# remit0/SpeechRecognitionProject

Measured on AMD Instinct MI355X. Metric: utterances/sec (1 s @16 kHz) MFCC+CNN-BiGRU train step, higher is better.
Workload: dtype fp32; 1 GPU; cfg2 mfcc_bgru: on-device MFCC[39x51] + 2-layer BiGRU(512) + FC, CE, backward, Adam (full training.py step), per-GPU batch 256; model=mfcc_bgru, global_batch=256, clip_samples=16000, parallelism=dp1, step_execution=HIP graph replay of the whole step, sync_bn=False

## Files before the change

include/srk.h:

```cpp
#ifndef SRK_H_
#define SRK_H_

#include <stdint.h>

#define SRK_ABI_VERSION 3

#ifdef __cplusplus
extern "C" {
#endif

enum srk_status {
  SRK_OK = 0,
  SRK_ERR_INVALID = -1,
  SRK_ERR_HIP = -2,
  SRK_ERR_INTERNAL = -3,
  SRK_ERR_TIMEOUT = -4,
};

int srk_version(void);
const char* srk_source_stamp(void);
const char* srk_last_error(void);
int srk_init(int device);
int64_t srk_scratch_generation(void);
int srk_prof_enable(int on);
// ... 54 lines not shown
                        float* rowsum, void* stream);
int srk_gemm_16(int trans_a, int trans_b, int64_t M, int64_t N, int64_t K, float alpha, const uint16_t* A,
                int64_t lda, const uint16_t* B, int64_t ldb, float beta, float* C, int64_t ldc,
                const float* bias, int bias_mode, void* stream);
int srk_gemm_16_batched(int trans_a, int trans_b, int64_t M, int64_t N, int64_t K, float alpha,
                        const uint16_t* A, int64_t lda, int64_t sA, const uint16_t* B, int64_t ldb,
                        int64_t sB, float beta, float* C, int64_t ldc, int64_t sC, int batch, void* stream);
int srk_colsum_f32(const float* X, int64_t M, int64_t N, int64_t ldx, float* out, float beta, void* stream);
int srk_gemm_plan_describe(int trans_a, int trans_b, int64_t M, int64_t N, int64_t K, int64_t lda, int64_t ldb,
                           int64_t ldc, int batch, int64_t sA, int64_t sB, int64_t sC, int bias_mode, int has_rowsum,
                           int operands16, int prec, int no_split, int plan_batch, uint64_t a_addr, uint64_t b_addr,
                           uint64_t c_addr, uint64_t bias_addr, char* buf, int64_t cap);
int srk_gemm_pack_plan(int64_t K, int64_t slab, int64_t first, int64_t stride, int64_t count, int64_t* blocks,
                       int64_t blocks_cap, int64_t* slab_counts, int64_t slabs_cap, int64_t* n_slabs,
                       int64_t* packed_slab);

int64_t srk_gru_workspace_floats(int64_t B, int64_t T, int64_t in, int64_t H, int backward);
int srk_gru_layer_fwd(const float* x, int64_t B, int64_t T, int64_t in, int64_t H, const float* w_ih,
                      const float* w_hh, const float* b_ih, const float* b_hh, float* y, float* ws,
                      void* stream);
int srk_gru_layer_bwd(const float* x, int64_t B, int64_t T, int64_t in, int64_t H, const float* w_ih,
                      const float* w_hh, const float* y, const float* ws_fwd, const float* dy, float* dx,
                      float* dw_ih, float* dw_hh, float* db_ih, float* db_hh, int accumulate, float* ws,
                      void* stream);
int64_t srk_gru_y16_offset(int64_t B, int64_t T, int64_t in, int64_t H);
int srk_gru_layer_fwd_x16(const float* x, const void* x16, int64_t B, int64_t T, int64_t in, int64_t H,
                          const float* w_ih, const float* w_hh, const float* b_ih, const float* b_hh, float* y,
                          float* ws, void* stream);
int srk_gru_layer_bwd_x16(const float* x, const void* x16, int64_t B, int64_t T, int64_t in, int64_t H,
                          const float* w_ih, const float* w_hh, const float* y, const float* ws_fwd, const float* dy,
// ... 157 lines not shown
```

speechrecognitionproject_amd/_lib.py:

```python
import contextlib
import ctypes
import os
import re

import torch

_HERE = os.path.dirname(os.path.abspath(__file__))
LIB_PATH = os.environ.get("SRK_LIB") or os.path.join(_HERE, "libsrk.so")
HEADER = os.path.join(os.path.dirname(_HERE), "include", "srk.h")
ABI_VERSION = 3

_P = ctypes.c_void_p
_I64 = ctypes.c_int64
_I = ctypes.c_int
_F = ctypes.c_float
_D = ctypes.c_double

_SIGS = {
    "srk_version": [],
    "srk_last_error": [],
    "srk_init": [_I],
    "srk_prof_enable": [_I],
    "srk_prof_read": [ctypes.c_char_p, ctypes.POINTER(ctypes.c_int64), ctypes.POINTER(ctypes.c_double),
                      ctypes.POINTER(ctypes.c_double)],
# ... 25 lines not shown
    "srk_augment": [_P, _I64, _P, _I64, _P, _P, _P, _P, ctypes.c_uint64, _P, _P],
    "srk_pitch_workspace_bytes": [_I64],
    "srk_pitch_shift": [_P, _I64, _P, _P, _I64, _P, _P, _I64, _P],
    "srk_wav_read_batch": [ctypes.POINTER(ctypes.c_char_p), _I64, _P, _P, _I],
    "srk_softmax_ensemble": [_P, _I64, _I64, _I64, _P, _P, _P, _P],
    "srk_gemm_f32": [_I, _I, _I64, _I64, _I64, _F, _P, _I64, _P, _I64, _F, _P, _I64, _P, _I, _P],
    "srk_gemm_rowsum_f32": [_I, _I, _I64, _I64, _I64, _F, _P, _I64, _P, _I64, _F, _P, _I64, _P, _P],
    "srk_gemm_16": [_I, _I, _I64, _I64, _I64, _F, _P, _I64, _P, _I64, _F, _P, _I64, _P, _I, _P],
    "srk_gemm_16_batched": [_I, _I, _I64, _I64, _I64, _F, _P, _I64, _I64, _P, _I64, _I64, _F, _P, _I64, _I64, _I, _P],
    "srk_colsum_f32": [_P, _I64, _I64, _I64, _P, _F, _P],
    "srk_gemm_plan_describe": [_I, _I, _I64, _I64, _I64, _I64, _I64, _I64, _I, _I64, _I64, _I64, _I, _I, _I, _I, _I, _I,
                               ctypes.c_uint64, ctypes.c_uint64, ctypes.c_uint64, ctypes.c_uint64, ctypes.c_char_p,
                               _I64],
    "srk_gemm_pack_plan": [_I64, _I64, _I64, _I64, _I64, ctypes.POINTER(_I64), _I64, ctypes.POINTER(_I64), _I64,
                           ctypes.POINTER(_I64), ctypes.POINTER(_I64)],
    "srk_gru_workspace_floats": [_I64, _I64, _I64, _I64, _I],
    "srk_gru_layer_fwd": [_P, _I64, _I64, _I64, _I64, _P, _P, _P, _P, _P, _P, _P],
    "srk_gru_layer_bwd": [_P, _I64, _I64, _I64, _I64, _P, _P, _P, _P, _P, _P, _P, _P, _P, _P, _I, _P, _P],
    "srk_gru_y16_offset": [_I64, _I64, _I64, _I64],
    "srk_gru_layer_fwd_x16": [_P, _P, _I64, _I64, _I64, _I64, _P, _P, _P, _P, _P, _P, _P],
    "srk_gru_layer_bwd_x16": [_P, _P, _I64, _I64, _I64, _I64, _P, _P, _P, _P, _P, _P, _P, _P, _P, _P, _I, _P, _P],
    "srk_gru_top_last_workspace_floats": [_I64, _I64, _I64, _I64, _I],
    "srk_gru_top_last_fwd": [_P, _P, _I64, _I64, _I64, _I64, _P, _P, _P, _P, _P, _P, _P, _P, _P],
    "srk_gru_top_last_bwd": [_P, _P, _I64, _I64, _I64, _I64, _P, _P, _P, _P, _P, _I, _P, _P, _P, _P, _P, _I, _P, _P],
    "srk_conv2d_workspace_floats": [_I64, _I64, _I64, _I64],
    "srk_conv2d_nhwc_fwd": [_P, _I64, _I64, _I64, _I64, _P, _P, _I64, _I64, _I64, _I64, _I64, _I64, _I64, _P, _P,
                            _P],
    "srk_conv2d_nhwc_bwd": [_P, _I64, _I64, _I64, _I64, _P, _I64, _I64, _I64, _I64, _I64, _I64, _I64, _P, _P, _P,
                            _P, _P, _P],
    "srk_conv2d_nhwc_fwd16": [_P, _I64, _I64, _I64, _I64, _P, _P, _I64, _I64, _I64, _I64, _I64, _I64, _I64, _P, _P,
# ... 129 lines not shown
def gemm_pack_plan(K, slab, first, stride, count):
    n = max(int(count), 0)
    ns = max(-(-int(K) // int(slab)), 0) if slab > 0 else 0
    blocks = (_I64 * max(n, 1))()
    counts = (_I64 * max(ns, 1))()
    n_slabs, pslab = _I64(0), _I64(0)
    call("srk_gemm_pack_plan", K, slab, first, stride, count, blocks, n, counts, ns, ctypes.byref(n_slabs),
         ctypes.byref(pslab))
    out, at = [], 0
    for s in range(n_slabs.value):
        out.append([int(b) for b in blocks[at:at + counts[s]]])
        at += counts[s]
    return out, int(pslab.value)


def scratch_generation():
    return int(lib().srk_scratch_generation())


PRECISIONS = {"fp32": 0, "bf16": 1, "fp16": 2}
_precision = "fp32"


def set_option(name, value):
    global _precision
    call("srk_set_option", name.encode(), int(value))
    if name == "matmul_precision":
        _precision = next(k for k, v in PRECISIONS.items() if v == int(value))


# ... 87 lines not shown
```

speechrecognitionproject_amd/csrc/gemm.h:

```cpp
#pragma once
#include "srk_internal.h"

namespace srk {

struct GemmDesc {
  int64_t M = 0, N = 0, K = 0;
  const float* A = nullptr; int64_t lda = 0; bool ta = false;
  const float* B = nullptr; int64_t ldb = 0; bool tb = false;
  float* C = nullptr; int64_t ldc = 0;
  float alpha = 1.f, beta = 0.f;
  const float* bias = nullptr; int bias_mode = 0;
  int batch = 1; int64_t sA = 0, sB = 0, sC = 0;
  float* rowsum = nullptr; float rowsum_beta = 0.f;
  int64_t sRS = 0;
  int prec = -1;
  const uint16_t* A16 = nullptr;
  const uint16_t* B16 = nullptr;
  bool no_split = false;
  int plan_batch = 0;
  int64_t plan_M = 0;
  int pin_splits = 0;
  int64_t pin_kchunk = 0;
};

int gemm_f32(const GemmDesc& d, hipStream_t stream);

bool gemm_f32_pin_as(const GemmDesc& full, GemmDesc& part);

bool gemm_f32_p32_split(const GemmDesc& d, int* splits, int64_t* kchunk);

constexpr int kGemmGroupMax = 4;
int gemm_f32_group(const GemmDesc* ds, int n, hipStream_t stream);
bool gemm_group_enabled();

struct PackPlan {
  int64_t K = 0, slab = 0, first = 0, stride = 0, count = 0;
  int64_t nslabs = 0, pslab = 0;
  __host__ __device__ int64_t lo(int64_t s) const {
    const int64_t k0 = s * slab;
    if (s >= nslabs) return count;
    if (k0 <= first) return 0;
    const int64_t b = (k0 - first + stride - 1) / stride;
    return b < count ? b : count;
  }
  __host__ __device__ int64_t src(int64_t kp, bool* live) const {
    const int64_t s = kp / pslab, r = kp - s * pslab, b = lo(s) + (r >> 3);
    *live = false;
    if (b >= lo(s + 1)) return -1;
// ... 15 lines not shown
```

speechrecognitionproject_amd/csrc/gemm.hip:

```cpp
#include <algorithm>
#include <cstdlib>
#include <type_traits>

#include "gemm.h"
#include "mfma_tile.h"

namespace srk {
namespace {

using namespace tile;

struct KernelArgs {
  GemmDesc d;
  int tiles_m, tiles_n;
  int tiles;
  int nblk;
  int group_m;
  int remap;
  int64_t kchunk;
  float* partial;
  float* rs_partial;
  int sk_wgs;
  int sk_ki;
  float* sk_slab;
};

__device__ __forceinline__ void tile_of(int t, int tiles_m, int tiles_n, int group_m, int& tm, int& tn) {
  const int gsz_full = group_m * tiles_n;
  const int grp = t / gsz_full, first_m = grp * group_m;
  const int gm = tiles_m - first_m < group_m ? tiles_m - first_m : group_m;
  const int tin = t - grp * gsz_full;
  tm = first_m + tin % gm;
  tn = tin / gm;
}
__device__ __forceinline__ int64_t sk_begin(int64_t w, int64_t total, int64_t W) { return w * total / W; }
__device__ __forceinline__ int sk_owner(int64_t it, int64_t total, int64_t W) { return (int)(((it + 1) * W - 1) / total); }

template <int TM, int TN>
__device__ __forceinline__ void store_acc(const KernelArgs& ka, const f32x16 (&acc)[TM][TN], int split, int64_t m0,
                                          int64_t n0, int wm0, int wn0, int lane, int64_t z) {
  const GemmDesc& d = ka.d;
  const int lh = lane >> 5, lc = lane & 31;
  const bool split_mode = ka.partial != nullptr;
#pragma unroll
  for (int i = 0; i < TM; ++i) {
#pragma unroll
    for (int j = 0; j < TN; ++j) {
      const int64_t col = n0 + wn0 + j * 32 + lc;
      if (col >= d.N) continue;
#pragma unroll
      for (int r = 0; r < 16; ++r) {
// ... 1081 lines not shown
  return ((double)d.M * (double)d.K * esz + (double)d.K * (double)d.N * esz + c) * (double)d.batch;
}

constexpr int kP32BK = 16;
template <bool KC>
struct P32Half {
  static constexpr int FLOATS = 128 * kP32BK;
  __device__ static __forceinline__ v4f frag(const float* img, int r0, int kb, int lane) {
    const int row = r0 + (lane & 31), h = lane >> 5;
    if (KC) return *reinterpret_cast<const v4f*>(img + row * kP32BK + (((2 * kb + h) ^ ((row >> 2) & 3)) << 2));
    const float* q = img + (8 * kb + 4 * h) * 128 + row;
    return v4f{q[0], q[128], q[256], q[384]};
  }
  __device__ static __forceinline__ void src(int piece, int lane, int64_t r0, int64_t rows, int64_t ld, unsigned& voff,
                                             int& kk, bool& row_ok) {
    const int p = piece * 64 + lane;
    if (KC) {
      const int row = p >> 2, kc = (p & 3) ^ ((row >> 2) & 3);
      voff = (unsigned)(((r0 + row) * ld + kc * 4) * 4);
      kk = kc * 4;
      row_ok = r0 + row < rows;
    } else {
      const int k = p >> 5, u = p & 31;
      voff = (unsigned)((k * ld + r0 + u * 4) * 4);
      kk = k;
      row_ok = r0 + u * 4 < rows;
    }
  }
  __device__ static __forceinline__ int64_t kstep_bytes(int64_t ld) { return KC ? 4 : 4 * ld; }
};

template <bool TA, bool TB>
__device__ __forceinline__ void gemm_p32_body(const KernelArgs& ka, const int blk, const int64_t z) {
  constexpr int BK = kP32BK, NST = 4;
  constexpr bool AKC = !TA, BKC = TB;
  using HA = P32Half<AKC>;
  using HB = P32Half<BKC>;
  constexpr int HALF = HA::FLOATS;
  constexpr int STAGE = 4 * HALF;
  __shared__ __attribute__((aligned(1024))) float smem[NST * STAGE];
  typedef __attribute__((address_space(3))) void* lds_ptr;
  auto bar = [] {
    asm volatile("" ::: "memory");
    __builtin_amdgcn_s_barrier();
    asm volatile("" ::: "memory");
// ... 7 lines not shown
    int lin = blk;
    if (ka.remap) {
      const int b = blk, xcd = b & 7, q = ka.nblk >> 3, r = ka.nblk & 7;
      lin = (xcd < r ? xcd * (q + 1) : r * (q + 1) + (xcd - r) * q) + (b >> 3);
    }
    sk_it = sk_begin(lin, sk_total, ka.sk_wgs);
    sk_end = sk_begin(lin + 1, sk_total, ka.sk_wgs);
  }
  for (bool first_seg = true;; first_seg = false) {
  int split = 0, tm, tn;
  int64_t kb0, ke;
  float* seg_slab = nullptr;
  if (sk) {
    if (sk_it >= sk_end) break;
    const int t = (int)(sk_it / ka.sk_ki);
    const int64_t t0 = (int64_t)t * ka.sk_ki, kt_end = min((int64_t)ka.sk_ki, sk_end - t0);
    kb0 = (sk_it - t0) * BK;
    ke = min(d.K, kt_end * BK);
    tile_of(t, ka.tiles_m, ka.tiles_n, ka.group_m, tm, tn);
    const int w0 = sk_owner(t0, sk_total, ka.sk_wgs), w1 = sk_owner(t0 + ka.sk_ki - 1, sk_total, ka.sk_wgs);
    const int wme = sk_owner(sk_it, sk_total, ka.sk_wgs);
    if (w1 > w0) seg_slab = ka.sk_slab + (int64_t)(wme - w0) * d.M * d.N;
    sk_it = t0 + ka.sk_ki;
    if (!first_seg) __syncthreads();
  } else {
    if (!first_seg) break;
    map_tile_at(blk, ka.nblk, ka.tiles, ka.tiles_m, ka.tiles_n, ka.group_m, ka.remap != 0, split, tm, tn);
    kb0 = split * ka.kchunk;
    ke = (kb0 + ka.kchunk < d.K) ? kb0 + ka.kchunk : d.K;
  }
  const int64_t m0 = (int64_t)tm * 256, n0 = (int64_t)tn * 256;
  const int nk = ke > kb0 ? (int)((ke - kb0 + BK - 1) / BK) : 0;

  typedef unsigned u32x4s __attribute__((ext_vector_type(4)));
  auto rsrc32 = [](const float* p) {
    const uint64_t a = (uint64_t)(uintptr_t)p;
    return u32x4s{(unsigned)__builtin_amdgcn_readfirstlane((unsigned)a),
                  (unsigned)__builtin_amdgcn_readfirstlane((unsigned)(a >> 32)), 0x7ffffff0u, 0x00020000u};
// ... 64 lines not shown
#pragma unroll
    for (int q = 0; q < BK / 8; ++q) {
      v4f fa[4], fb[2];
#pragma unroll
      for (int i = 0; i < 4; ++i) fa[i] = HA::frag(As, i * 32, q, lane);
#pragma unroll
      for (int j = 0; j < 2; ++j) fb[j] = HB::frag(Bs, bc0 + j * 32, q, lane);
      if (tn_ < nk) {
        if (q == 0) dma_a(tn_);
        else dma_b(tn_);
      }
      if (q == BK / 8 - 1) retire_keep(min(nk - 1 - (kt + 1), NST - 2));
      asm volatile("s_waitcnt lgkmcnt(0)" ::: "memory");
      bar();
      __builtin_amdgcn_s_setprio(1);
#pragma unroll
      for (int ss = 0; ss < 4; ++ss)
#pragma unroll
        for (int i = 0; i < 4; ++i)
#pragma unroll
          for (int j = 0; j < 2; ++j) acc[i][j] = __builtin_amdgcn_mfma_f32_32x32x2f32(fa[i][ss], fb[j][ss], acc[i][j], 0, 0, 0);
      __builtin_amdgcn_s_setprio(0);
      if (do_rs) {
#pragma unroll
        for (int i = 0; i < 4; ++i) rs[i] += (fa[i][0] + fa[i][1]) + (fa[i][2] + fa[i][3]);
      }
      bar();
    }
  }
  if (grp == 0) bar();

  pp_epilogue(ka, acc, smem, split, m0, n0, grp, wc, wave, lane, z, seg_slab);
  if (do_rs) {
    const int splits = ka.nblk / ka.tiles;
    float* rsum = d.rowsum + z * d.sRS;
#pragma unroll
// ... 24 lines not shown
  const int b = (int)blockIdx.x;
  int i = 0;
#pragma unroll
  for (int j = 1; j < kGemmGroupMax; ++j)
    if (j < ga.n && b >= ga.first[j]) i = j;
  const int blk = b - ga.first[i];
  if (blk >= ga.m[i].nblk) return;
  gemm_p32_body<TA, TB>(ga.m[i], blk, 0);
}

constexpr int kSkFixupSlices = 8;
__global__ __launch_bounds__(256) void sk_fixup_kernel(KernelArgs ka) {
  const GemmDesc& d = ka.d;
  const int t = blockIdx.x / kSkFixupSlices, slice = blockIdx.x - t * kSkFixupSlices;
  const int64_t total = (int64_t)ka.tiles * ka.sk_ki, t0 = (int64_t)t * ka.sk_ki;
  const int w0 = sk_owner(t0, total, ka.sk_wgs), w1 = sk_owner(t0 + ka.sk_ki - 1, total, ka.sk_wgs);
  if (w1 == w0) return;
  int tm, tn;
  tile_of(t, ka.tiles_m, ka.tiles_n, ka.group_m, tm, tn);
  const int nseg = w1 - w0 + 1;
  const int64_t MN = d.M * d.N;
  const bool vec = d.N % 4 == 0 && d.ldc % 4 == 0 && (uintptr_t)d.C % 16 == 0 && (uintptr_t)ka.sk_slab % 16 == 0 &&
                   (d.bias_mode != 1 || (uintptr_t)d.bias % 16 == 0);
  constexpr int ROWS = 256 / kSkFixupSlices, ITEMS = ROWS * 64 / 256;
  const int64_t r0 = (int64_t)tm * 256 + slice * ROWS;
  if (vec) {
    v4f v[ITEMS];
    int64_t off[ITEMS];
    bool ok[ITEMS];
#pragma unroll
    for (int u = 0; u < ITEMS; ++u) {
// ... 30 lines not shown
    const int64_t row = r0 + (i >> 6), col = (int64_t)tn * 256 + (i & 63) * 4;
    if (row >= d.M || col >= d.N) continue;
    const int64_t o = row * d.N + col;
#pragma unroll
    for (int e = 0; e < 4; ++e) {
      if (col + e >= d.N) break;
      float v = 0.f;
      for (int g = 0; g < nseg; ++g) v += ka.sk_slab[g * MN + o + e];
      v *= d.alpha;
      if (d.bias_mode == 1) v += d.bias[col + e];
      else if (d.bias_mode == 2) v += d.bias[row];
      float* c = d.C + row * d.ldc + col + e;
      if (d.beta != 0.f) v += d.beta * *c;
      *c = v;
    }
  }
}

__global__ __launch_bounds__(256) void splitk_reduce_kernel(GemmDesc d, const float* __restrict__ partial, int splits) {
  const int64_t i = (int64_t)blockIdx.x * blockDim.x + threadIdx.x;
  if (i >= d.M * d.N) return;
  partial += (int64_t)blockIdx.y * splits * d.M * d.N;
  d.C += (int64_t)blockIdx.y * d.sC;
  const int64_t row = i / d.N, col = i % d.N;
  float s = 0.f;
#pragma unroll 8
  for (int k = 0; k < splits; ++k) s += partial[(int64_t)k * d.M * d.N + i];
  float v = d.alpha * s;
  if (d.bias_mode == 1) v += d.bias[col];
  else if (d.bias_mode == 2) v += d.bias[row];
// ... 477 lines not shown
  part.pin_kchunk = pf.ka.kchunk;
  if (gemm_plan(part, pp) == SRK_OK && pp.family == pf.family && pp.bk == pf.bk && pp.prec == pf.prec) return true;
  part.pin_splits = 0;
  part.pin_kchunk = 0;
  return false;
}

bool gemm_f32_p32_split(const GemmDesc& d, int* splits, int64_t* kchunk) {
  GemmPlan p;
  if (gemm_plan(d, p) != SRK_OK || p.family != kFamP32 || p.streamk) return false;
  *splits = p.splits;
  *kchunk = p.ka.kchunk;
  return true;
}

int gemm_f32_group(const GemmDesc* ds, int n, hipStream_t s) {
  SRK_REQUIRE(ds && n >= 1 && n <= kGemmGroupMax, SRK_ERR_INVALID, "gemm_group: 1 .. %d members", kGemmGroupMax);
  GemmPlan plans[kGemmGroupMax];
  int order[kGemmGroupMax];
  for (int i = 0; i < n; ++i) {
    if (int rc = gemm_plan(ds[i], plans[i])) return rc;
    SRK_REQUIRE(plans[i].family == kFamP32 && !plans[i].streamk && ds[i].batch == 1 && ds[i].ta == ds[0].ta &&
                    ds[i].tb == ds[0].tb,
                SRK_ERR_INVALID, "gemm_group: member %d is not a batch-1, non-stream-K gemm_p32_kernel launch of the "
                "group's (ta, tb)", i);
    order[i] = i;
  }
  const auto klen = [&](int i) { return std::min(plans[i].ka.kchunk, std::max<int64_t>(ds[i].K, 1)); };
  std::stable_sort(order, order + n, [&](int a, int b) { return klen(a) > klen(b); });
  size_t off[kGemmGroupMax], need = 0;
// ... 162 lines not shown
    for (int64_t r = 0; r < p.pslab; r += 8) {
      bool live;
      const int64_t row = p.src(s * p.pslab + r, &live);
      if (row < 0) continue;
      SRK_REQUIRE(nb < blocks_cap, SRK_ERR_INTERNAL, "gemm_pack_plan: more kept blocks than live rows");
      blocks[nb++] = row / 8;
      ++slab_counts[s];
    }
  }
  *n_slabs = p.nslabs;
  *packed_slab = p.pslab;
  return SRK_OK;
  SRK_API_END
}

extern "C" int srk_gemm_plan_describe(int trans_a, int trans_b, int64_t M, int64_t N, int64_t K, int64_t lda,
                                      int64_t ldb, int64_t ldc, int batch, int64_t sA, int64_t sB, int64_t sC,
                                      int bias_mode, int has_rowsum, int operands16, int prec, int no_split,
                                      int plan_batch, uint64_t a_addr, uint64_t b_addr, uint64_t c_addr,
                                      uint64_t bias_addr, char* buf, int64_t cap) {
  SRK_API_BEGIN
  SRK_REQUIRE(buf && cap > 0, SRK_ERR_INVALID, "gemm_plan_describe: no buffer");
  buf[0] = 0;
  srk::GemmDesc d;
  d.M = M; d.N = N; d.K = K;
  d.lda = lda; d.ta = trans_a != 0;
  d.ldb = ldb; d.tb = trans_b != 0;
  if (operands16) {
    d.A16 = reinterpret_cast<const uint16_t*>(a_addr); d.B16 = reinterpret_cast<const uint16_t*>(b_addr);
  } else {
// ... 18 lines not shown
```

speechrecognitionproject_amd/csrc/gru.hip:

```cpp
#include <algorithm>

#include "gemm.h"
#include "gru_internal.h"

namespace srk {
namespace {

constexpr int kRows = 64;
constexpr int kUnits = 16;
constexpr int kBK = 128;
constexpr int kPitch = kBK + 4;

struct GruArgs {
  int B, T, H, in;
  int G, S;
  const float* y_in;
  float* y;
  const float* gi;
  const float* w_hh;
  const float* b_hh;
  float* gates;
  const float* dy;
  float* dgi;
  float* dgh;
// ... 698 lines not shown
  const int64_t ld = h16 ? in8_of(in) : srk::pad4(in);
  const bool pad = ld != in;
  float* wpad = pad && !h16 ? ws + L.wpad : nullptr;
  float* dwpad = pad ? ws + (h16 ? L.dwpad8 : L.dwpad) : nullptr;
  float* dxpad = pad ? ws + (h16 ? L.dxpad8 : L.dxpad) : nullptr;
  Mat m_dgi{dgi, nullptr}, m_dgh{dgh, nullptr}, m_x{pad ? ws_fwd + F.xpad : x, nullptr},
      m_w{pad ? wpad : w_ih, nullptr}, m_y{y, nullptr};
  if (h16) {
    m_dgi = {nullptr, u16(ws + L.dgi)};
    m_dgh = {nullptr, u16(ws + L.dgh16)};
    m_x = {nullptr, x16_in ? static_cast<const uint16_t*>(x16_in) : u16(ws_fwd + F.x16)};
    m_w = {nullptr, u16(ws_fwd + F.w16)};
    m_y = {nullptr, u16(ws_fwd + F.y16)};
  }
  int rc;
  const int dw_parts = h16 ? path.bwd.dw_parts : 0;
  if (path.persistent) {
    srk::GruPArgs p = rec_args(B, T, H, w_hh, ws, L);
    p.y_in = y; p.gates = gates; p.dy = dy;
    if (h16) {
      p.dgi16 = const_cast<uint16_t*>(m_dgi.h); p.dgh16 = const_cast<uint16_t*>(m_dgh.h); p.dbias = ws + L.part;
      if (dw_parts) {
        if ((rc = srk::g_gs.get((size_t)dw_parts * 2 * 3 * H * H, &p.dw_part))) return rc;
        p.y16_in = m_y.h;
      }
    } else {
      p.dgi = dgi; p.dgh = dgh; p.dgh_edge = dgh_edge;
      p.one_dir = top_last >= 2 ? 1 : 0;
    }
    if ((rc = srk::gru_persistent_launch(p, path.bwd, true, s))) return rc;
    if (h16) {
      const int prows = path.bwd.bias_part_rows, bparts = (int)((B + 255) / 256 * (256 / prows));
      if (dw_parts) {
        const int64_t per_dir = 3 * H * H, n4 = 2 * per_dir / 4;
        const int dw_blocks = (int)((n4 + 255) / 256);
        srk::ProfScope prof("gru_dwhh_reduce", s, 4.0 * (dw_parts + 2) * 2 * per_dir);
        hipLaunchKernelGGL(srk::dwhh_dbias_reduce_kernel, dim3((unsigned)(dw_blocks + (6 * H + 255) / 256)), dim3(256),
                           0, s, p.dw_part, dw_parts, (int)B, per_dir, dw_hh, (int)accumulate, dw_blocks, p.dbias,
                           bparts, (int)H, prows, db_ih, db_hh);
        SRK_CHECK_HIP(hipGetLastError());
      } else if ((rc = srk::launch256(srk::dbias_reduce_kernel, 6 * H, s, p.dbias, bparts, B, H, prows, db_ih, db_hh,
                                      accumulate))) {
        return rc;
      }
    }
    if (top_last == 3 && (rc = srk::launch256(srk::zero_cols_kernel, BT * 3 * H / 4, s, dgi, BT, 3 * H, 3 * H, 6 * H)))
      return rc;
    if (top_last >= 2 && (rc = srk::launch256(srk::rev_cell_bwd_kernel, B * H, s, gates, dy_last, B, T, H, dgi, dgh_edge)))
      return rc;
  } else {
    srk::GruArgs a{};
    a.B = (int)B; a.T = (int)T; a.H = (int)H; a.in = (int)in;
    a.y_in = y; a.w_hh = w_hh; a.gates = gates;
    a.dy = dy; a.dgi = dgi; a.dgh = dgh; a.dgh_edge = dgh_edge; a.dhz = ws + L.dhz;
    a.G = (int)((B + srk::kRows - 1) / srk::kRows);
    a.S = (int)(H / srk::kUnits);
    const dim3 grid((unsigned)(2 * a.G * a.S));
    for (int step = 0; step < T; ++step) {
      srk::ProfScope prof("gru_bwd_step", s, step > 0 ? 2.0 * 2.0 * (double)B * 3 * H * H : 0.0);
      hipLaunchKernelGGL(srk::gru_bwd_step_kernel, grid, dim3(256), 0, s, a, step);
    }
    SRK_CHECK_HIP(hipGetLastError());
  }

  const float beta = accumulate ? 1.f : 0.f;
  const bool sums = !h16;
  const bool rev_last = top_last == 1 || top_last == 2;
  const Mat m_dgi_rev = m_dgi.at((T - 1) * 6 * H + 3 * H);
  bool grouped = false;
  if (top_last == 3 && !h16 && T >= 16 && srk::gemm_group_enabled()) {
    GemmDesc full;
    full.M = 6 * H; full.N = ld; full.K = BT;
    full.A = dgi; full.lda = 6 * H; full.ta = true;
    full.B = m_x.f; full.ldb = ld;
    full.C = pad ? dwpad : dw_ih; full.ldc = ld; full.beta = pad ? 0.f : beta;
    full.rowsum = db_ih; full.rowsum_beta = beta;
    GemmDesc hh;
    hh.M = 3 * H; hh.N = H; hh.K = BT - 1;
    hh.ta = true; hh.lda = 3 * H; hh.ldb = 2 * H;
    hh.A = dgh + 3 * H; hh.B = y;
    hh.C = dw_hh; hh.ldc = H; hh.beta = beta;
    hh.batch = 2; hh.sA = BT * 3 * H - 3 * H; hh.sB = 3 * H; hh.sC = 3 * H * H;
    hh.rowsum = db_hh; hh.rowsum_beta = beta; hh.sRS = 3 * H;
    int splits = 0;
    int64_t kchunk = 0;
    srk::PackPlan pp;
    if (srk::gemm_f32_p32_split(full, &splits, &kchunk) && splits > 1 && srk::g_opt_gru_dwhh_batched &&
        srk::gemm_f32_batched_rowsum_ok(hh) && srk::pack_plan(BT, kchunk, T - 1, T, B, pp) == SRK_OK &&
        pp.nslabs == splits) {
      grouped = true;
      const int64_t rows = pp.nslabs * pp.pslab;
      float* packed = nullptr;
      if ((rc = srk::g_gs.get((size_t)rows * (3 * H + ld), &packed))) return rc;
      if ((rc = srk::gemm_pack_rows(pp, dgi + 3 * H, 6 * H, 3 * H, m_x.f, ld, ld, packed, packed + rows * 3 * H, s)))
        return rc;
      GemmDesc m[3];
      m[0] = full;
      m[0].M = 3 * H; m[0].plan_M = 6 * H;
      m[1] = hh;
      m[1].batch = 1; m[1].plan_batch = 2;
      m[2] = m[0];
      m[2].K = rows; m[2].pin_splits = (int)pp.nslabs; m[2].pin_kchunk = pp.pslab;
      m[2].A = packed; m[2].lda = 3 * H;
      m[2].B = packed + rows * 3 * H;
      m[2].C = full.C + 3 * H * ld;
      m[2].rowsum = db_ih + 3 * H;
      if ((rc = srk::gemm_f32_group(m, 3, s))) return rc;
      if (pad && (rc = srk::launch256(srk::unpad_cols_kernel, 6 * H * in, s, dwpad, 6 * H, ld, dw_ih, in, accumulate)))
        return rc;
      if (!accumulate) {
        SRK_CHECK_HIP(hipMemsetAsync(dw_hh + 3 * H * H, 0, sizeof(float) * 3 * H * H, s));
        SRK_CHECK_HIP(hipMemsetAsync(db_hh + 3 * H, 0, sizeof(float) * 3 * H, s));
      }
    }
  }
  if (!grouped) {
    GemmDesc g;
    g.M = rev_last ? 3 * H : 6 * H; g.N = ld; g.K = BT;
    set_a(g, m_dgi); g.lda = 6 * H; g.ta = true;
    set_b(g, m_x); g.ldb = ld;
    g.C = pad ? dwpad : dw_ih; g.ldc = ld; g.beta = pad ? 0.f : beta;
    if (sums) { g.rowsum = db_ih; g.rowsum_beta = beta; }
    if ((rc = srk::gemm_f32(g, s))) return rc;
    if (rev_last) {
      g.K = B;
      set_a(g, m_dgi_rev); g.lda = T * 6 * H;
      set_b(g, m_x.at((T - 1) * ld)); g.ldb = T * ld;
      g.C += 3 * H * g.ldc;
// ... 42 lines not shown
    } else if (!accumulate) {
      SRK_CHECK_HIP(hipMemsetAsync(dw_hh, 0, sizeof(float) * 2 * 3 * H * H, s));
      if (sums) SRK_CHECK_HIP(hipMemsetAsync(db_hh, 0, sizeof(float) * 2 * 3 * H, s));
    }
  }
  if (sums)
    for (int dir = 0; dir < 2; ++dir)
      if ((rc = srk::colsum_f32(dgh_edge + (size_t)dir * B * 3 * H, B, 3 * H, 3 * H, db_hh + dir * 3 * H, 1.f, s)))
        return rc;
  if (dx) {
    if (h16 && in <= srk::kFusedIn) {
      if ((rc = srk::to16(w_ih, 6 * H, in, const_cast<uint16_t*>(m_w.h), ld, s))) return rc;
    } else if (!h16 && pad) {
      if ((rc = srk::pad_cols(w_ih, 6 * H, in, wpad, s))) return rc;
    }
    GemmDesc g;
    g.M = BT; g.N = ld; g.K = rev_last ? 3 * H : 6 * H;
    set_a(g, m_dgi); g.lda = 6 * H;
    set_b(g, m_w); g.ldb = ld;
    g.C = pad ? dxpad : dx; g.ldc = ld;
    if ((rc = srk::gemm_f32(g, s))) return rc;
    if (rev_last) {
      g.M = B;
      set_a(g, m_dgi_rev); g.lda = T * 6 * H;
      set_b(g, m_w.at(3 * H * ld));
      g.C += (T - 1) * g.ldc; g.ldc *= T;
      g.beta = 1.f;
      if ((rc = srk::gemm_f32(g, s))) return rc;
    }
    if (pad && (rc = srk::launch256(srk::unpad_cols_kernel, BT * in, s, dxpad, BT, ld, dx, in, 0))) return rc;
  }
  return SRK_OK;
}

int srk_gru_layer_bwd_x16(const float* x, const void* x16_in, int64_t B, int64_t T, int64_t in, int64_t H,
                          const float* w_ih, const float* w_hh, const float* y, const float* ws_fwd, const float* dy,
// ... 33 lines not shown
```

Before: 59270 utt/s.

## Add k-live stream-K GEMM for GRU dx to skip zero reverse-gate columns

```diff
diff --git a/include/srk.h b/include/srk.h
--- a/include/srk.h
+++ b/include/srk.h
@@ -92,6 +92,12 @@
 int srk_gemm_pack_plan(int64_t K, int64_t slab, int64_t first, int64_t stride, int64_t count, int64_t* blocks,
                        int64_t blocks_cap, int64_t* slab_counts, int64_t slabs_cap, int64_t* n_slabs,
                        int64_t* packed_slab);
+int srk_gemm_f32_klive(int64_t M, int64_t N, int64_t K, const float* A, int64_t lda, const float* B, int64_t ldb,
+                       float* C, int64_t ldc, int64_t k_live, int64_t first, int64_t stride, int64_t count,
+                       void* stream);
+int srk_gemm_klive_plan(int64_t M, int64_t N, int64_t K, int64_t k_live, int64_t first, int64_t stride, int64_t count,
+                        float beta, int bias_mode, int64_t* kept, int64_t kept_cap, int64_t* live_runs,
+                        int64_t runs_cap, int64_t* tiles, int64_t* ktiles, int64_t* wgs);
 
 int64_t srk_gru_workspace_floats(int64_t B, int64_t T, int64_t in, int64_t H, int backward);
 int srk_gru_layer_fwd(const float* x, int64_t B, int64_t T, int64_t in, int64_t H, const float* w_ih,
diff --git a/speechrecognitionproject_amd/_lib.py b/speechrecognitionproject_amd/_lib.py
--- a/speechrecognitionproject_amd/_lib.py
+++ b/speechrecognitionproject_amd/_lib.py
@@ -63,6 +63,10 @@
                                _I64],
     "srk_gemm_pack_plan": [_I64, _I64, _I64, _I64, _I64, ctypes.POINTER(_I64), _I64, ctypes.POINTER(_I64), _I64,
                            ctypes.POINTER(_I64), ctypes.POINTER(_I64)],
+    "srk_gemm_f32_klive": [_I64, _I64, _I64, _P, _I64, _P, _I64, _P, _I64, _I64, _I64, _I64, _I64, _P],
+    "srk_gemm_klive_plan": [_I64, _I64, _I64, _I64, _I64, _I64, _I64, _F, _I, ctypes.POINTER(_I64), _I64,
+                            ctypes.POINTER(_I64), _I64, ctypes.POINTER(_I64), ctypes.POINTER(_I64),
+                            ctypes.POINTER(_I64)],
     "srk_gru_workspace_floats": [_I64, _I64, _I64, _I64, _I],
     "srk_gru_layer_fwd": [_P, _I64, _I64, _I64, _I64, _P, _P, _P, _P, _P, _P, _P],
     "srk_gru_layer_bwd": [_P, _I64, _I64, _I64, _I64, _P, _P, _P, _P, _P, _P, _P, _P, _P, _P, _I, _P, _P],
@@ -222,6 +226,15 @@
     return out, int(pslab.value)
 
 
+def gemm_klive_plan(M, N, K, k_live, first, stride, count, beta=0.0, bias_mode=0):
+    nt = max(-(-int(M) // 256) * -(-int(N) // 256), 1)
+    kept, runs = (_I64 * 1024)(), (_I64 * nt)()
+    tiles, ktiles, wgs = _I64(0), _I64(0), _I64(0)
+    call("srk_gemm_klive_plan", M, N, K, k_live, first, stride, count, beta, bias_mode, kept, 1024, runs, nt,
+         ctypes.byref(tiles), ctypes.byref(ktiles), ctypes.byref(wgs))
+    return tiles.value, ktiles.value, [int(k) for k in kept[:wgs.value]], [int(r) for r in runs[:tiles.value]]
+
+
 def scratch_generation():
     return int(lib().srk_scratch_generation())
 
diff --git a/speechrecognitionproject_amd/csrc/gemm.h b/speechrecognitionproject_amd/csrc/gemm.h
--- a/speechrecognitionproject_amd/csrc/gemm.h
+++ b/speechrecognitionproject_amd/csrc/gemm.h
@@ -21,6 +21,7 @@
   int64_t plan_M = 0;
   int pin_splits = 0;
   int64_t pin_kchunk = 0;
+  int64_t k_live = 0, live_first = 0, live_stride = 0, live_count = 0;
 };
 
 int gemm_f32(const GemmDesc& d, hipStream_t stream);
@@ -32,6 +33,10 @@
 constexpr int kGemmGroupMax = 4;
 int gemm_f32_group(const GemmDesc* ds, int n, hipStream_t stream);
 bool gemm_group_enabled();
+
+bool gemm_f32_klive_ok(const GemmDesc& d);
+int gemm_f32_klive(const GemmDesc& d, hipStream_t stream);
+bool gemm_klive_enabled();
 
 struct PackPlan {
   int64_t K = 0, slab = 0, first = 0, stride = 0, count = 0;
diff --git a/speechrecognitionproject_amd/csrc/gemm.hip b/speechrecognitionproject_amd/csrc/gemm.hip
--- a/speechrecognitionproject_amd/csrc/gemm.hip
+++ b/speechrecognitionproject_amd/csrc/gemm.hip
@@ -23,7 +23,9 @@
   int sk_wgs;
   int sk_ki;
   float* sk_slab;
+  int live_ki;
 };
+__host__ __device__ __forceinline__ int sk_live(const KernelArgs& ka) { return ka.live_ki > 0 ? ka.live_ki : ka.sk_ki; }
 
 __device__ __forceinline__ void tile_of(int t, int tiles_m, int tiles_n, int group_m, int& tm, int& tn) {
   const int gsz_full = group_m * tiles_n;
@@ -33,8 +35,8 @@
   tm = first_m + tin % gm;
   tn = tin / gm;
 }
-__device__ __forceinline__ int64_t sk_begin(int64_t w, int64_t total, int64_t W) { return w * total / W; }
-__device__ __forceinline__ int sk_owner(int64_t it, int64_t total, int64_t W) { return (int)(((it + 1) * W - 1) / total); }
+__host__ __device__ __forceinline__ int64_t sk_begin(int64_t w, int64_t total, int64_t W) { return w * total / W; }
+__host__ __device__ __forceinline__ int sk_owner(int64_t it, int64_t total, int64_t W) { return (int)(((it + 1) * W - 1) / total); }
 
 template <int TM, int TN>
 __device__ __forceinline__ void store_acc(const KernelArgs& ka, const f32x16 (&acc)[TM][TN], int split, int64_t m0,
@@ -1146,21 +1148,32 @@
   }
   __device__ static __forceinline__ void src(int piece, int lane, int64_t r0, int64_t rows, int64_t ld, unsigned& voff,
                                              int& kk, bool& row_ok) {
-    const int p = piece * 64 + lane;
+    int row;
+    unit(piece * 64 + lane, row, kk);
+    voff = (unsigned)((KC ? (r0 + row) * ld + kk : kk * ld + r0 + row) * 4);
+    row_ok = r0 + row < rows;
+  }
+  __device__ static __forceinline__ void unit(int p, int& row, int& kk) {
     if (KC) {
-      const int row = p >> 2, kc = (p & 3) ^ ((row >> 2) & 3);
-      voff = (unsigned)(((r0 + row) * ld + kc * 4) * 4);
-      kk = kc * 4;
-      row_ok = r0 + row < rows;
+      row = p >> 2;
+      kk = ((p & 3) ^ ((row >> 2) & 3)) * 4;
     } else {
-      const int k = p >> 5, u = p & 31;
-      voff = (unsigned)((k * ld + r0 + u * 4) * 4);
-      kk = k;
-      row_ok = r0 + u * 4 < rows;
+      kk = p >> 5;
+      row = (p & 31) * 4;
     }
   }
   __device__ static __forceinline__ int64_t kstep_bytes(int64_t ld) { return KC ? 4 : 4 * ld; }
 };
+
+template <int TM, int TN>
+__device__ __forceinline__ void p32_mma_block(const v4f (&fa)[TM], const v4f (&fb)[TN], f32x16 (&acc)[TM][TN]) {
+#pragma unroll
+  for (int ss = 0; ss < 4; ++ss)
+#pragma unroll
+    for (int i = 0; i < TM; ++i)
+#pragma unroll
+      for (int j = 0; j < TN; ++j) acc[i][j] = __builtin_amdgcn_mfma_f32_32x32x2f32(fa[i][ss], fb[j][ss], acc[i][j], 0, 0, 0);
+}
 
 template <bool TA, bool TB>
 __device__ __forceinline__ void gemm_p32_body(const KernelArgs& ka, const int blk, const int64_t z) {
@@ -1198,14 +1211,16 @@
   if (sk) {
     if (sk_it >= sk_end) break;
     const int t = (int)(sk_it / ka.sk_ki);
-    const int64_t t0 = (int64_t)t * ka.sk_ki, kt_end = min((int64_t)ka.sk_ki, sk_end - t0);
-    kb0 = (sk_it - t0) * BK;
+    const int64_t t0 = (int64_t)t * ka.sk_ki, live = sk_live(ka), kt_end = min(live, sk_end - t0);
+    const int64_t it0 = sk_it;
+    sk_it = t0 + ka.sk_ki;
+    if (it0 - t0 >= live) continue;
+    kb0 = (it0 - t0) * BK;
     ke = min(d.K, kt_end * BK);
     tile_of(t, ka.tiles_m, ka.tiles_n, ka.group_m, tm, tn);
-    const int w0 = sk_owner(t0, sk_total, ka.sk_wgs), w1 = sk_owner(t0 + ka.sk_ki - 1, sk_total, ka.sk_wgs);
-    const int wme = sk_owner(sk_it, sk_total, ka.sk_wgs);
+    const int w0 = sk_owner(t0, sk_total, ka.sk_wgs), w1 = sk_owner(t0 + live - 1, sk_total, ka.sk_wgs);
+    const int wme = sk_owner(it0, sk_total, ka.sk_wgs);
     if (w1 > w0) seg_slab = ka.sk_slab + (int64_t)(wme - w0) * d.M * d.N;
-    sk_it = t0 + ka.sk_ki;
     if (!first_seg) __syncthreads();
   } else {
     if (!first_seg) break;
@@ -1300,12 +1315,7 @@
       asm volatile("s_waitcnt lgkmcnt(0)" ::: "memory");
       bar();
       __builtin_amdgcn_s_setprio(1);
-#pragma unroll
-      for (int ss = 0; ss < 4; ++ss)
-#pragma unroll
-        for (int i = 0; i < 4; ++i)
-#pragma unroll
-          for (int j = 0; j < 2; ++j) acc[i][j] = __builtin_amdgcn_mfma_f32_32x32x2f32(fa[i][ss], fb[j][ss], acc[i][j], 0, 0, 0);
+      p32_mma_block(fa, fb, acc);
       __builtin_amdgcn_s_setprio(0);
       if (do_rs) {
 #pragma unroll
@@ -1360,7 +1370,7 @@
   const GemmDesc& d = ka.d;
   const int t = blockIdx.x / kSkFixupSlices, slice = blockIdx.x - t * kSkFixupSlices;
   const int64_t total = (int64_t)ka.tiles * ka.sk_ki, t0 = (int64_t)t * ka.sk_ki;
-  const int w0 = sk_owner(t0, total, ka.sk_wgs), w1 = sk_owner(t0 + ka.sk_ki - 1, total, ka.sk_wgs);
+  const int w0 = sk_owner(t0, total, ka.sk_wgs), w1 = sk_owner(t0 + sk_live(ka) - 1, total, ka.sk_wgs);
   if (w1 == w0) return;
   int tm, tn;
   tile_of(t, ka.tiles_m, ka.tiles_n, ka.group_m, tm, tn);
@@ -1421,6 +1431,104 @@
       if (d.beta != 0.f) v += d.beta * *c;
       *c = v;
     }
+  }
+}
+
+constexpr int kLiveKT = 2;
+template <bool TB>
+__global__ __launch_bounds__(512, 1) void p32_live_rows_kernel(KernelArgs ka) {
+  constexpr int BK = kP32BK, KT = kLiveKT;
+  using HA = P32Half<true>;
+  using HB = P32Half<TB>;
+  constexpr int AIMG = 32 * BK;
+  constexpr int TILE = AIMG + 2 * HB::FLOATS;
+  constexpr int NB = KT * 2 * (HB::FLOATS / 4) / 512;
+  static_assert(KT * (AIMG / 4) <= 512 && NB * 512 == KT * 2 * (HB::FLOATS / 4), "staging must divide evenly");
+  __shared__ __attribute__((aligned(16))) float smem[2 * KT * TILE];
+  const GemmDesc& d = ka.d;
+  const int tid = threadIdx.x, lane = tid & 63, wave = tid >> 6;
+  const int t = blockIdx.x;
+  int tm, tn;
+  tile_of(t, ka.tiles_m, ka.tiles_n, ka.group_m, tm, tn);
+  const int64_t m0 = (int64_t)tm * 256, m1 = min(m0 + 256, d.M), n0 = (int64_t)tn * 256;
+  const int64_t j0 = m0 <= d.live_first ? 0 : (m0 - d.live_first + d.live_stride - 1) / d.live_stride;
+  if (m1 <= d.live_first || j0 >= d.live_count) return;
+  const int64_t j1 = min(d.live_count - 1, (m1 - 1 - d.live_first) / d.live_stride);
+  const int nlive = (int)min((int64_t)32, j1 - j0 + 1);
+  if (nlive <= 0) return;
+  const int64_t total = (int64_t)ka.tiles * ka.sk_ki, t0 = (int64_t)t * ka.sk_ki;
+  const int w0 = sk_owner(t0, total, ka.sk_wgs), w1 = sk_owner(t0 + ka.sk_ki - 1, total, ka.sk_wgs);
+  const int cut1 = w1 > w0 ? (int)(sk_begin(w0 + 1, total, ka.sk_wgs) - t0) : -1;
+  const int cut2 = w1 > w0 + 1 ? (int)(sk_begin(w0 + 2, total, ka.sk_wgs) - t0) : -1;
+
+  v4f ra, rb[NB];
+  const v4f zero4 = v4f{0.f, 0.f, 0.f, 0.f};
+  auto load_stage = [&](int st) {
+    if (tid < KT * (AIMG / 4)) {
+      int row, kk;
+      HA::unit(tid % (AIMG / 4), row, kk);
+      const int64_t k = ((int64_t)st * KT + tid / (AIMG / 4)) * BK + kk;
+      ra = row < nlive && k < d.K ? ld4(d.A + (d.live_first + (j0 + row) * d.live_stride) * d.lda + k) : zero4;
+    }
+#pragma unroll
+    for (int i = 0; i < NB; ++i) {
+      const int e = tid + 512 * i, u = e % (HB::FLOATS / 4), half = (e / (HB::FLOATS / 4)) & 1;
+      int row, kk;
+      HB::unit(u, row, kk);
+      const int64_t k = ((int64_t)st * KT + e / (2 * (HB::FLOATS / 4))) * BK + kk, n = n0 + half * 128 + row;
+      const bool ok = n < d.N && k < d.K;
+      rb[i] = ok ? ld4(TB ? d.B + n * d.ldb + k : d.B + k * d.ldb + n) : zero4;
+    }
+  };
+  auto store_stage = [&](int buf) {
+    float* S = smem + buf * (KT * TILE);
+    if (tid < KT * (AIMG / 4)) st4(S + (tid / (AIMG / 4)) * TILE + (tid % (AIMG / 4)) * 4, ra);
+#pragma unroll
+    for (int i = 0; i < NB; ++i) {
+      const int e = tid + 512 * i;
+      st4(S + (e / (2 * (HB::FLOATS / 4))) * TILE + AIMG + (e % (2 * (HB::FLOATS / 4))) * 4, rb[i]);
+    }
+  };
+
+  f32x16 acc[1][1], sum;
+#pragma unroll
+  for (int r = 0; r < 16; ++r) acc[0][0][r] = sum[r] = 0.f;
+  int nrun = 0;
+  const int bh = wave >> 2, c0 = (wave & 3) * 32;
+  const int nstage = (ka.sk_ki + KT - 1) / KT;
+  load_stage(0);
+  store_stage(0);
+  __syncthreads();
+  for (int st = 0; st < nstage; ++st) {
+    if (st + 1 < nstage) load_stage(st + 1);
+    const float* S = smem + (st & 1) * (KT * TILE);
+#pragma unroll
+    for (int kt = 0; kt < KT; ++kt) {
+      const int g = st * KT + kt;
+      if (g >= ka.sk_ki) break;
+      if (g == cut1 || g == cut2) {
+        sum = nrun ? sum + acc[0][0] : acc[0][0];
+        ++nrun;
+#pragma unroll
+        for (int r = 0; r < 16; ++r) acc[0][0][r] = 0.f;
+      }
+#pragma unroll
+      for (int q = 0; q < BK / 8; ++q) {
+        const v4f fa[1] = {HA::frag(S + kt * TILE, 0, q, lane)};
+        const v4f fb[1] = {HB::frag(S + kt * TILE + AIMG + bh * HB::FLOATS, c0, q, lane)};
+        p32_mma_block(fa, fb, acc);
+      }
+    }
+    if (st + 1 < nstage) store_stage((st + 1) & 1);
+    __syncthreads();
+  }
+  const f32x16 out = nrun ? sum + acc[0][0] : acc[0][0];
+  const int64_t col = n0 + bh * 128 + c0 + (lane & 31);
+  if (col >= d.N) return;
+#pragma unroll
+  for (int r = 0; r < 16; ++r) {
+    const int i = (r & 3) + 8 * (r >> 2) + 4 * (lane >> 5);
+    if (i < nlive) d.C[(d.live_first + (j0 + i) * d.live_stride) * d.ldc + col] = out[r];
   }
 }
 
@@ -1928,6 +2036,62 @@
   return true;
 }
 
+bool gemm_klive_enabled() {
+  static const bool on = [] {
+    const char* v = getenv("SRK_GEMM_KLIVE");
+    return !(v && *v) || atoi(v) != 0;
+  }();
+  return on;
+}
+
+namespace {
+bool klive_plan(const GemmDesc& d, GemmPlan& p) {
+  if (d.k_live <= 0 || d.k_live % kP32BK != 0 || d.k_live >= d.K || d.live_count < 1 || d.live_first < 0 ||
+      d.live_stride < 8 || d.live_count > d.M || d.live_first + (d.live_count - 1) * d.live_stride >= d.M)
+    return false;
+  if (d.ta || d.batch != 1 || d.alpha != 1.f || d.beta != 0.f || d.bias_mode != 0 || d.rowsum || d.A16 || d.B16) return false;
+  if (gemm_plan(d, p) != SRK_OK || p.family != kFamP32 || !p.streamk || p.prec != kPrecF32) return false;
+  p.ka.live_ki = (int)(d.k_live / kP32BK);
+  p.flops = 2.0 * (double)d.M * (double)d.N * (double)d.k_live;
+  return true;
+}
+}
+
+bool gemm_f32_klive_ok(const GemmDesc& d) {
+  GemmPlan p;
+  return klive_plan(d, p);
+}
+
+int gemm_f32_klive(const GemmDesc& d, hipStream_t s) {
+  GemmPlan p;
+  SRK_REQUIRE(klive_plan(d, p), SRK_ERR_INVALID,
+              "gemm_klive: needs the fp32 stream-K gemm_p32_kernel plan (A not transposed, batch 1, alpha 1, beta 0, no bias, "
+              "no row sums), k_live a multiple of %d in (0, K), live rows below M at a stride >= 8", kP32BK);
+  float* scratch = nullptr;
+  if (int rc = g_scratch.get(plan_scratch(p), &scratch)) return rc;
+  const KernelArgs ka = plan_args(p, d, scratch);
+  {
+    ProfScope prof(p.name, s, p.flops);
+    prof.bytes(p.bytes - 4.0 * (double)d.M * (double)(d.K - d.k_live));
+    if (prof.on()) {
+      char detail[96];
+      gemm_plan_detail(p, d, detail);
+      prof.detail("%s klive %lld", detail, (long long)d.k_live);
+    }
+    hipLaunchKernelGGL(p.kernel, p.grid, p.block, 0, s, ka);
+    hipLaunchKernelGGL(sk_fixup_kernel, dim3((unsigned)ka.tiles * kSkFixupSlices), dim3(256), 0, s, ka);
+    SRK_CHECK_HIP(hipGetLastError());
+  }
+  ProfScope prof(p.name, s, 2.0 * 32 * 256 * (double)ka.tiles * (double)d.K);
+  if (prof.on())
+    prof.detail("p32_live_rows_kernel<N%c> %lldx%lldx%lld rows %lld", d.tb ? 'T' : 'N', (long long)d.M, (long long)d.N,
+                (long long)d.K, (long long)d.live_count);
+  if (d.tb) hipLaunchKernelGGL(p32_live_rows_kernel<true>, dim3((unsigned)ka.tiles), dim3(512), 0, s, ka);
+  else hipLaunchKernelGGL(p32_live_rows_kernel<false>, dim3((unsigned)ka.tiles), dim3(512), 0, s, ka);
+  SRK_CHECK_HIP(hipGetLastError());
+  return SRK_OK;
+}
+
 int gemm_f32_group(const GemmDesc* ds, int n, hipStream_t s) {
   SRK_REQUIRE(ds && n >= 1 && n <= kGemmGroupMax, SRK_ERR_INVALID, "gemm_group: 1 .. %d members", kGemmGroupMax);
   GemmPlan plans[kGemmGroupMax];
@@ -2120,6 +2284,61 @@
   SRK_API_END
 }
 
+extern "C" int srk_gemm_f32_klive(int64_t M, int64_t N, int64_t K, const float* A, int64_t lda, const float* B,
+                                  int64_t ldb, float* C, int64_t ldc, int64_t k_live, int64_t first, int64_t stride,
+                                  int64_t count, void* stream) {
+  SRK_API_BEGIN
+  srk::GemmDesc d;
+  d.M = M; d.N = N; d.K = K;
+  d.A = A; d.lda = lda;
+  d.B = B; d.ldb = ldb;
+  d.C = C; d.ldc = ldc;
+  d.k_live = k_live; d.live_first = first; d.live_stride = stride; d.live_count = count;
+  return srk::gemm_f32_klive(d, srk::as_stream(stream));
+  SRK_API_END
+}
+
+extern "C" int srk_gemm_klive_plan(int64_t M, int64_t N, int64_t K, int64_t k_live, int64_t first, int64_t stride,
+                                   int64_t count, float beta, int bias_mode, int64_t* kept, int64_t kept_cap,
+                                   int64_t* live_runs, int64_t runs_cap, int64_t* tiles, int64_t* ktiles,
+                                   int64_t* wgs) {
+  SRK_API_BEGIN
+  SRK_REQUIRE(kept && live_runs && tiles && ktiles && wgs && kept_cap >= 0 && runs_cap >= 0, SRK_ERR_INVALID,
+              "gemm_klive_plan: null pointer");
+  srk::GemmDesc d;
+  d.M = M; d.N = N; d.K = K;
+  d.A = reinterpret_cast<const float*>(uintptr_t(256)); d.lda = K;
+  d.B = reinterpret_cast<const float*>(uintptr_t(256)); d.ldb = N;
+  d.C = reinterpret_cast<float*>(uintptr_t(256)); d.ldc = N;
+  d.beta = beta;
+  d.bias_mode = bias_mode; d.bias = bias_mode ? reinterpret_cast<const float*>(uintptr_t(256)) : nullptr;
+  d.k_live = k_live; d.live_first = first; d.live_stride = stride; d.live_count = count;
+  srk::GemmPlan p;
+  SRK_REQUIRE(srk::klive_plan(d, p), SRK_ERR_INVALID, "gemm_klive_plan: not a case of gemm_f32_klive");
+  const srk::KernelArgs& ka = p.ka;
+  SRK_REQUIRE(kept_cap >= ka.sk_wgs && runs_cap >= ka.tiles, SRK_ERR_INVALID,
+              "gemm_klive_plan: need room for %d workgroups and %d tiles", ka.sk_wgs, ka.tiles);
+  const int64_t total = (int64_t)ka.tiles * ka.sk_ki, live = srk::sk_live(ka);
+  for (int w = 0; w < ka.sk_wgs; ++w) {
+    kept[w] = 0;
+    const int64_t end = srk::sk_begin(w + 1, total, ka.sk_wgs);
+    for (int64_t it = srk::sk_begin(w, total, ka.sk_wgs); it < end;) {
+      const int64_t t0 = it / ka.sk_ki * ka.sk_ki, kt_end = std::min(live, end - t0);
+      if (it - t0 < live) kept[w] += kt_end - (it - t0);
+      it = t0 + ka.sk_ki;
+    }
+  }
+  for (int t = 0; t < ka.tiles; ++t) {
+    const int64_t t0 = (int64_t)t * ka.sk_ki;
+    live_runs[t] = srk::sk_owner(t0 + live - 1, total, ka.sk_wgs) - srk::sk_owner(t0, total, ka.sk_wgs) + 1;
+  }
+  *tiles = ka.tiles;
+  *ktiles = ka.sk_ki;
+  *wgs = ka.sk_wgs;
+  return SRK_OK;
+  SRK_API_END
+}
+
 extern "C" int srk_gemm_plan_describe(int trans_a, int trans_b, int64_t M, int64_t N, int64_t K, int64_t lda,
                                       int64_t ldb, int64_t ldc, int batch, int64_t sA, int64_t sB, int64_t sC,
                                       int bias_mode, int has_rowsum, int operands16, int prec, int no_split,
diff --git a/speechrecognitionproject_amd/csrc/gru.hip b/speechrecognitionproject_amd/csrc/gru.hip
--- a/speechrecognitionproject_amd/csrc/gru.hip
+++ b/speechrecognitionproject_amd/csrc/gru.hip
@@ -736,6 +736,39 @@
     m_y = {nullptr, u16(ws_fwd + F.y16)};
   }
   int rc;
+  const float beta = accumulate ? 1.f : 0.f;
+  bool grouped = false;
+  GemmDesc full, hh;
+  srk::PackPlan pp;
+  if (top_last == 3 && !h16 && T >= 16 && srk::gemm_group_enabled()) {
+    full.M = 6 * H; full.N = ld; full.K = BT;
+    full.A = dgi; full.lda = 6 * H; full.ta = true;
+    full.B = m_x.f; full.ldb = ld;
+    full.C = pad ? dwpad : dw_ih; full.ldc = ld; full.beta = pad ? 0.f : beta;
+    full.rowsum = db_ih; full.rowsum_beta = beta;
+    hh.M = 3 * H; hh.N = H; hh.K = BT - 1;
+    hh.ta = true; hh.lda = 3 * H; hh.ldb = 2 * H;
+    hh.A = dgh + 3 * H; hh.B = y;
+    hh.C = dw_hh; hh.ldc = H; hh.beta = beta;
+    hh.batch = 2; hh.sA = BT * 3 * H - 3 * H; hh.sB = 3 * H; hh.sC = 3 * H * H;
+    hh.rowsum = db_hh; hh.rowsum_beta = beta; hh.sRS = 3 * H;
+    int splits = 0;
+    int64_t kchunk = 0;
+    grouped = srk::gemm_f32_p32_split(full, &splits, &kchunk) && splits > 1 && srk::g_opt_gru_dwhh_batched &&
+              srk::gemm_f32_batched_rowsum_ok(hh) && srk::pack_plan(BT, kchunk, T - 1, T, B, pp) == SRK_OK &&
+              pp.nslabs == splits;
+  }
+  GemmDesc gdx;
+  gdx.M = BT; gdx.N = ld; gdx.K = (top_last == 1 || top_last == 2) ? 3 * H : 6 * H;
+  set_a(gdx, m_dgi); gdx.lda = 6 * H;
+  set_b(gdx, m_w); gdx.ldb = ld;
+  gdx.C = pad ? dxpad : dx; gdx.ldc = ld;
+  bool dx_klive = false;
+  if (dx && top_last == 3 && !h16 && srk::gemm_klive_enabled()) {
+    gdx.k_live = 3 * H; gdx.live_first = T - 1; gdx.live_stride = T; gdx.live_count = B;
+    dx_klive = srk::gemm_f32_klive_ok(gdx);
+    if (!dx_klive) gdx.k_live = 0;
+  }
   const int dw_parts = h16 ? path.bwd.dw_parts : 0;
   if (path.persistent) {
     srk::GruPArgs p = rec_args(B, T, H, w_hh, ws, L);
@@ -766,7 +799,8 @@
         return rc;
       }
     }
-    if (top_last == 3 && (rc = srk::launch256(srk::zero_cols_kernel, BT * 3 * H / 4, s, dgi, BT, 3 * H, 3 * H, 6 * H)))
+    const bool rev_unread = grouped && (!dx || dx_klive);
+    if (top_last == 3 && !rev_unread && (rc = srk::launch256(srk::zero_cols_kernel, BT * 3 * H / 4, s, dgi, BT, 3 * H, 3 * H, 6 * H)))
       return rc;
     if (top_last >= 2 && (rc = srk::launch256(srk::rev_cell_bwd_kernel, B * H, s, gates, dy_last, B, T, H, dgi, dgh_edge)))
       return rc;
@@ -785,55 +819,32 @@
     SRK_CHECK_HIP(hipGetLastError());
   }
 
-  const float beta = accumulate ? 1.f : 0.f;
   const bool sums = !h16;
   const bool rev_last = top_last == 1 || top_last == 2;
   const Mat m_dgi_rev = m_dgi.at((T - 1) * 6 * H + 3 * H);
-  bool grouped = false;
-  if (top_last == 3 && !h16 && T >= 16 && srk::gemm_group_enabled()) {
-    GemmDesc full;
-    full.M = 6 * H; full.N = ld; full.K = BT;
-    full.A = dgi; full.lda = 6 * H; full.ta = true;
-    full.B = m_x.f; full.ldb = ld;
-    full.C = pad ? dwpad : dw_ih; full.ldc = ld; full.beta = pad ? 0.f : beta;
-    full.rowsum = db_ih; full.rowsum_beta = beta;
-    GemmDesc hh;
-    hh.M = 3 * H; hh.N = H; hh.K = BT - 1;
-    hh.ta = true; hh.lda = 3 * H; hh.ldb = 2 * H;
-    hh.A = dgh + 3 * H; hh.B = y;
-    hh.C = dw_hh; hh.ldc = H; hh.beta = beta;
-    hh.batch = 2; hh.sA = BT * 3 * H - 3 * H; hh.sB = 3 * H; hh.sC = 3 * H * H;
-    hh.rowsum = db_hh; hh.rowsum_beta = beta; hh.sRS = 3 * H;
-    int splits = 0;
-    int64_t kchunk = 0;
-    srk::PackPlan pp;
-    if (srk::gemm_f32_p32_split(full, &splits, &kchunk) && splits > 1 && srk::g_opt_gru_dwhh_batched &&
-        srk::gemm_f32_batched_rowsum_ok(hh) && srk::pack_plan(BT, kchunk, T - 1, T, B, pp) == SRK_OK &&
-        pp.nslabs == splits) {
-      grouped = true;
-      const int64_t rows = pp.nslabs * pp.pslab;
-      float* packed = nullptr;
-      if ((rc = srk::g_gs.get((size_t)rows * (3 * H + ld), &packed))) return rc;
-      if ((rc = srk::gemm_pack_rows(pp, dgi + 3 * H, 6 * H, 3 * H, m_x.f, ld, ld, packed, packed + rows * 3 * H, s)))
-        return rc;
-      GemmDesc m[3];
-      m[0] = full;
-      m[0].M = 3 * H; m[0].plan_M = 6 * H;
-      m[1] = hh;
-      m[1].batch = 1; m[1].plan_batch = 2;
-      m[2] = m[0];
-      m[2].K = rows; m[2].pin_splits = (int)pp.nslabs; m[2].pin_kchunk = pp.pslab;
-      m[2].A = packed; m[2].lda = 3 * H;
-      m[2].B = packed + rows * 3 * H;
-      m[2].C = full.C + 3 * H * ld;
-      m[2].rowsum = db_ih + 3 * H;
-      if ((rc = srk::gemm_f32_group(m, 3, s))) return rc;
-      if (pad && (rc = srk::launch256(srk::unpad_cols_kernel, 6 * H * in, s, dwpad, 6 * H, ld, dw_ih, in, accumulate)))
-        return rc;
-      if (!accumulate) {
-        SRK_CHECK_HIP(hipMemsetAsync(dw_hh + 3 * H * H, 0, sizeof(float) * 3 * H * H, s));
-        SRK_CHECK_HIP(hipMemsetAsync(db_hh + 3 * H, 0, sizeof(float) * 3 * H, s));
-      }
+  if (grouped) {
+    const int64_t rows = pp.nslabs * pp.pslab;
+    float* packed = nullptr;
+    if ((rc = srk::g_gs.get((size_t)rows * (3 * H + ld), &packed))) return rc;
+    if ((rc = srk::gemm_pack_rows(pp, dgi + 3 * H, 6 * H, 3 * H, m_x.f, ld, ld, packed, packed + rows * 3 * H, s)))
+      return rc;
+    GemmDesc m[3];
+    m[0] = full;
+    m[0].M = 3 * H; m[0].plan_M = 6 * H;
+    m[1] = hh;
+    m[1].batch = 1; m[1].plan_batch = 2;
+    m[2] = m[0];
+    m[2].K = rows; m[2].pin_splits = (int)pp.nslabs; m[2].pin_kchunk = pp.pslab;
+    m[2].A = packed; m[2].lda = 3 * H;
+    m[2].B = packed + rows * 3 * H;
+    m[2].C = full.C + 3 * H * ld;
+    m[2].rowsum = db_ih + 3 * H;
+    if ((rc = srk::gemm_f32_group(m, 3, s))) return rc;
+    if (pad && (rc = srk::launch256(srk::unpad_cols_kernel, 6 * H * in, s, dwpad, 6 * H, ld, dw_ih, in, accumulate)))
+      return rc;
+    if (!accumulate) {
+      SRK_CHECK_HIP(hipMemsetAsync(dw_hh + 3 * H * H, 0, sizeof(float) * 3 * H * H, s));
+      SRK_CHECK_HIP(hipMemsetAsync(db_hh + 3 * H, 0, sizeof(float) * 3 * H, s));
     }
   }
   if (!grouped) {
@@ -906,12 +917,8 @@
     } else if (!h16 && pad) {
       if ((rc = srk::pad_cols(w_ih, 6 * H, in, wpad, s))) return rc;
     }
-    GemmDesc g;
-    g.M = BT; g.N = ld; g.K = rev_last ? 3 * H : 6 * H;
-    set_a(g, m_dgi); g.lda = 6 * H;
-    set_b(g, m_w); g.ldb = ld;
-    g.C = pad ? dxpad : dx; g.ldc = ld;
-    if ((rc = srk::gemm_f32(g, s))) return rc;
+    GemmDesc g = gdx;
+    if ((rc = dx_klive ? srk::gemm_f32_klive(g, s) : srk::gemm_f32(g, s))) return rc;
     if (rev_last) {
       g.M = B;
       set_a(g, m_dgi_rev); g.lda = T * 6 * H;
```

Measured after the change: 60730 utt/s (median of 6 runs). +2.5%, better.
